# KolinGuo/MPlib

Measured on AMD Instinct MI355X. Metric: configs/sec full collide() Panda-7DoF+10 boxes, higher is better.
Workload: dtype f64; 1 GPU; cfg3 panda_10boxes: 1048576 configs/GPU/step, 129 pairs, full self+world collide() with ACM filter; configs_per_gpu=1048576, pairs=129, mask_words=5, parallelism=dp1 (config shards, no data-path collective)

## Files before the change

### mplib_amd/csrc/mpg_kernels.hip

```cpp

#include <hip/hip_runtime.h>

#include <algorithm>
#include <atomic>
#include <chrono>
#include <cfloat>
#include <cstdio>
#include <cstdlib>
#include <cstring>
#include <limits>
#include <map>
#include <memory>
#include <mutex>
#include <string>
#include <thread>
#include <vector>

#include "../../include/mpgpu.h"
#include "mpg_math.h"
#include "mpg_fk.h"
#include "mpg_hostpipe.h"

using namespace mpg;

namespace {


thread_local std::string g_last_error;

int set_error(int code, const std::string& msg) {
  g_last_error = msg;
  return code;
}

#define HIP_TRY(expr)                                                                 \
  do {                                                                                \
    hipError_t _e = (expr);                                                           \
    if (_e != hipSuccess)                                                             \
      return set_error(MPG_E_HIP, std::string(#expr " failed: ") + hipGetErrorString(_e)); \
  } while (0)




struct GObj {
  CQ4 rot, rot_inv;
  CV3 pos;
  int geom;
  int type;
};

__device__ __forceinline__ V3 hull_vertex(const DevWorld& w, cptr<double> HV, int geom, int i) {
  const cptr<double> G = HV + 12 * (size_t)(w.geom_gstart[geom] + (i >> 2)) + (i & 3);
  return v3(G[0], G[4], G[8]);
}

__device__ __forceinline__ double edot(const V3& d, const V3& p) { return (d.x * p.x + d.y * p.y) + d.z * p.z; }

__device__ __forceinline__ V3 convex_full_scan(const DevWorld& w, cptr<double> HV, int geom, const V3& dir) {
  const int g0 = w.geom_gstart[geom], ng = w.geom_ng[geom];
  const cptr<double> P = HV + 12 * (size_t)g0;
  double best = -DBL_MAX;
  int bi = 0;
  for (int g = 0; g < ng; ++g) {
    const cptr<double> G = P + 12 * g;
    double dd[4];
#pragma unroll
    for (int k = 0; k < 4; ++k) dd[k] = (dir.x * G[k] + dir.y * G[4 + k]) + dir.z * G[8 + k];
#pragma unroll
    for (int k = 0; k < 4; ++k)
      if (dd[k] > best) {
        best = dd[k];
        bi = 4 * g + k;
      }
  }
  const cptr<double> B = P + 12 * (bi >> 2) + (bi & 3);
  return v3(B[0], B[4], B[8]);
}

constexpr int kWalkWords = kMaxWalkVerts / 64;
struct WalkScratch {
  uint64_t vis[kWalkWords];
  double dd[64];
  int vi[64];
};

__device__ __forceinline__ WalkScratch& walk_scratch() {
  __shared__ WalkScratch s_walk[8];
  return s_walk[(threadIdx.x >> 6) & 7];
}

__device__ __forceinline__ void wave_lds_sync() {
  __builtin_amdgcn_fence(__ATOMIC_SEQ_CST, "wavefront");
  __builtin_amdgcn_wave_barrier();
}

__device__ __forceinline__ double lane_bcast(double v, int L) {
  const unsigned long long u = (unsigned long long)__double_as_longlong(v);
  const unsigned lo = (unsigned)__builtin_amdgcn_readlane((int)(unsigned)u, L);
  const unsigned hi = (unsigned)__builtin_amdgcn_readlane((int)(unsigned)(u >> 32), L);
  return __longlong_as_double((long long)(((unsigned long long)hi << 32) | lo));
}

__device__ __forceinline__ int big_vis_acquire(const DevWorld& w, int rank) {
  int slot = 0;
  if (rank == 0) {
    const int n = w.big_slots;
    int k = (int)((blockIdx.x * 8u + (threadIdx.x >> 6)) % (unsigned)n);
    while (atomicCAS(&w.big_busy[k], 0, 1) != 0) k = k + 1 == n ? 0 : k + 1;
    slot = k;
  }
  return __builtin_amdgcn_readfirstlane(slot);
}

__device__ __forceinline__ int wave_walk(const DevWorld& w, cptr<double> HV, int geom, const V3& d, int rank,
                                         int nact, cptr<int> pre) {
  WalkScratch& S = walk_scratch();
  const cptr<int> hd = w.hull_nbr + 2 * w.geom_nbr[geom];
  const int nwords = (w.geom_nvert[geom] + 63) >> 6;
  const bool big = nwords > kWalkWords;
  const int slot = big ? big_vis_acquire(w, rank) : -1;
  unsigned long long* vis = big ? w.big_vis + (size_t)slot * w.big_words : (unsigned long long*)S.vis;
  if (big) {
    if (rank == 0) atomicOr(&vis[0], 1ull);
    __threadfence();
  } else {
    for (int j = rank; j < nwords; j += nact)
      S.vis[j] = pre ? (uint64_t)(uint32_t)pre[4 + 2 * j] | ((uint64_t)(uint32_t)pre[5 + 2 * j] << 32) : (j == 0 ? 1ull : 0ull);
  }
  wave_lds_sync();
  int bi = pre ? pre[0] : 0, pv = pre ? pre[1] : 0, k0 = pre ? pre[2] : 0;
  bool keep = pre ? pre[3] != 0 : false, first = true;
  double best = edot(d, hull_vertex(w, HV, geom, bi));
  do {
    const int v = first ? pv : bi;
    const int skip = first ? k0 : 0;
    bool moved = first && keep;
    first = false;
    const int start = hd[2 * v] + skip, cnt = hd[2 * v + 1] - skip;
    for (int c0 = 0; c0 < cnt; c0 += nact) {
      const int m = min(cnt - c0, nact);
      if (rank < m) {
        const cptr<double> e = w.nbr_ent + 4 * (size_t)(start + c0 + rank);
        const int vi = (int)e[3];
        const uint64_t bit = 1ull << (vi & 63);
        const bool seen = (atomicOr(&vis[vi >> 6], (unsigned long long)bit) & bit) != 0ull;
        S.vi[rank] = seen ? -1 : vi;
        S.dd[rank] = seen ? 0.0 : (d.x * e[0] + d.y * e[1]) + d.z * e[2];
      }
      wave_lds_sync();
      for (int k = 0; k < m; ++k) {
        const int vi = S.vi[k];
        const double dd = S.dd[k];
        if (vi >= 0 && dd >= best) {
          moved = true;
          bi = vi;
          best = dd;
        }
      }
      wave_lds_sync();
    }
    bi = __builtin_amdgcn_readfirstlane(bi);
    keep = moved;
  } while (keep);
  if (big) {
    for (int j = rank; j < nwords; j += nact) atomicExch(&vis[j], 0ull);
    __threadfence();
    wave_lds_sync();
    if (rank == 0) atomicExch(&w.big_busy[slot], 0);
  }
  return bi;
}

// ... 799 lines not shown
    const int nk = w.n_links - w.n_free;
    for (int l = 0; l < nk; ++l) {
      const double* pl = in + (c * w.n_links + l) * 7;
      forced |= !(std::fabs(pl[0]) <= w.pose_bound && std::fabs(pl[1]) <= w.pose_bound && std::fabs(pl[2]) <= w.pose_bound);
    }
    for (int k = 0; k < w.n_free; ++k) {
      const double* pl = in + (c * w.n_links + nk + k) * 7;
      const int m = w.free_obj[k];
      const cptr<double> gr = w.geom_rec + G_STRIDE * w.moving_geom[m];
      double R[9];
      quat_to_mat(pl[3], pl[4], pl[5], pl[6], R);
      double d2 = 0.0;
#pragma unroll
      for (int i = 0; i < 3; ++i) {
        const double ci = R[3 * i] * gr[G_OBB_C] + R[3 * i + 1] * gr[G_OBB_C + 1] + R[3 * i + 2] * gr[G_OBB_C + 2] + pl[i];
        d2 += ci * ci;
      }
      if (std::sqrt(d2) - gr[G_RADIUS] > w.far_r) {
        float* r = cen + (size_t)m * 3 * BLOCK + tid;
        r[0] = kFarPark;
        r[BLOCK] = 0.f;
        r[2 * BLOCK] = 0.f;
      }
    }
  } else {
    bp_fk(w.bp, in + c * w.dof, save + tid, BLOCK, put_j);
    if (w.n_prism)
      for (int j = 0; j < w.nj; ++j)
        if (w.prism_bound[j] >= 0.0) forced |= !(std::fabs(in[c * w.dof + w.joint_q_source[j]]) <= w.prism_bound[j]);
  }
  if (w.dbg(1) || w.dbg(13)) {
    if (live && cen[tid] == 12345.f) flags[cfg] = 2;
    return;
  }

  uint32_t head = 0, tail = 0;
  uint32_t dbg_keep = 0u;
  auto push = [&](int eb, uint32_t kb) {
    if (!live) kb = 0u;
    if (w.dbg(11)) {
      dbg_keep += kb;
      return;
    }
    if (w.dbg(2)) {
      for (int i = 0; i < 32; ++i) {
        if (!((kb >> i) & 1u)) continue;
        const int p = w.sched_pair[eb + i];
        survw[(p >> 5) * BLOCK + tid] |= 1u << (p & 31);
      }
      return;
    }
    {
    const uint32_t c = (uint32_t)__popc(kb);
    uint32_t ex = 0u, total = 0u;
#pragma unroll
    for (int bit = 0; bit < 6; ++bit) {
      const unsigned long long m = __ballot((c >> bit) & 1u);
      ex += __builtin_amdgcn_mbcnt_hi((uint32_t)(m >> 32), __builtin_amdgcn_mbcnt_lo((uint32_t)m, 0u)) << bit;
      total += (uint32_t)__popcll(m) << bit;
    }
    const uint32_t incl = ex + c;
    if (total == 0u) return;
    if (tail - head + total <= (uint32_t)kQueue) {
      uint32_t pos = tail + incl - c;
      while (kb) {
        const int i = __builtin_ctz(kb);
        kb &= kb - 1u;
        queue[pos++ & (kQueue - 1)] = ((uint32_t)(eb + i) << 6) | lane;
      }
      tail += total;
      while (tail - head >= 64) {
        sat_drain<BLOCK>(w, cen, rq, cap, cfg0, survw, queue, head, 64, wbase, lane);
        head += 64;
      }
      return;
    }
    }
    uint32_t any_kb = kb;
#pragma unroll
    for (int sh = 1; sh < 64; sh <<= 1) any_kb |= (uint32_t)__shfl_xor((int)any_kb, sh);
    any_kb = __builtin_amdgcn_readfirstlane(any_kb);
    while (any_kb) {
      const int i = __builtin_ctz(any_kb);
      any_kb &= any_kb - 1u;
      const bool keep = (kb >> i) & 1u;
      const unsigned long long bal = __ballot(keep);
      if (keep) {
        const uint32_t rank =
            __builtin_amdgcn_mbcnt_hi((uint32_t)(bal >> 32), __builtin_amdgcn_mbcnt_lo((uint32_t)bal, 0u));
        queue[(tail + rank) & (kQueue - 1)] = ((uint32_t)(eb + i) << 6) | lane;
      }
      tail += (uint32_t)__popcll(bal);
      if (tail - head >= 64) {
        sat_drain<BLOCK>(w, cen, rq, cap, cfg0, survw, queue, head, 64, wbase, lane);
        head += 64;
      }
    }
  };
  const int ns = w.n_static;
  for (int g = 0; g < (FROM_POSES ? 2 : 1) && !w.dbg(12); ++g) {
    const int E0 = w.st_start[g * (ns + 1)], E1 = w.st_start[g * (ns + 1) + ns];
    if (E0 == E1) continue;
    int eb = E0;
    uint32_t kb = 0u;
    for (int sid = 0; sid < ns; ++sid) {
      const int e0 = w.st_start[g * (ns + 1) + sid], e1 = w.st_start[g * (ns + 1) + sid + 1];
      if (e0 == e1) continue;
      const cptr<float> rec = w.bp.sobj + BS_STRIDE * sid;
      float sr[BS_STRIDE];
#pragma unroll
      for (int k = 0; k < BS_STRIDE; ++k) sr[k] = rec[k];
#pragma unroll 2
      for (int e = e0; e < e1; ++e) {
        if (e - eb == 32) {
          push(eb, kb);
          eb = e;
          kb = 0u;
        }
        const float* rm = cen + (size_t)w.st_m[e] * 3 * BLOCK + tid;
        const float cm[3] = {rm[0], rm[BLOCK], rm[2 * BLOCK]};
        kb |= (uint32_t)!fsphere_obb_separated(cm, w.st_r[e], sr, w.bp_margin) << (e - eb);
      }
    }
    push(eb, kb);
  }
  for (int m = 0; m < w.n_moving; ++m) {
    const int e0 = w.sched_start[m], e1 = w.sched_start[m + 1];
    if (e0 == e1) continue;
    const float* rm = cen + (size_t)m * 3 * BLOCK + tid;
    const float cm[3] = {rm[0], rm[BLOCK], rm[2 * BLOCK]};
    const float r_m = w.bp.mobj[BM_STRIDE * m + BM_R];
    for (int eb = e0; eb < e1; eb += 32) {
      const int ee = min(e1, eb + 32);
      uint32_t kb = 0u;
#pragma unroll 4
      for (int e = eb; e < ee; ++e) {
        const int o = w.sched_other[e];
        const float* ro = cen + (size_t)o * 3 * BLOCK + tid;
        const float dx = ro[0] - cm[0], dy = ro[BLOCK] - cm[1], dz = ro[2 * BLOCK] - cm[2];
        const float rr = r_m + w.bp.mobj[BM_STRIDE * o + BM_R] + w.bp_margin;
        kb |= (uint32_t)(dx * dx + dy * dy + dz * dz <= rr * rr) << (e - eb);
      }
      push(eb, kb);
    }
  }
  if (tail != head) sat_drain<BLOCK>(w, cen, rq, cap, cfg0, survw, queue, head, tail - head, wbase, lane);
  if (forced)
    for (int k = 0; k < w.W; ++k) survw[k * BLOCK + tid] = (uint32_t)w.all_mask[k];
  if (w.dbg(8) || w.dbg(11)) {
    if (live && (survw[tid] == 12345u || dbg_keep == 12345u)) flags[cfg] = 2;
    return;
  }
  bool any = false;
  const long long tile = (cfg0 >> 6) + (tid >> 6);
  if (w.W * 8 <= kQueue) {
    uint32_t* hist = queue;
    for (int i = (int)lane; i < w.W * 8; i += 64) hist[i] = 0u;
    wave_lds_sync();
    for (int k = 0; k < w.W; ++k) {
      uint32_t x = live ? survw[k * BLOCK + tid] : 0u;
      if (live) surv[(long long)k * cap + cfg] = x;
      any |= x != 0u;
      while (x) {
        const int p = k * 32 + __builtin_ctz(x);
        x &= x - 1u;
        atomicAdd(&hist[p >> 2], 1u << (8 * (p & 3)));
      }
    }
    wave_lds_sync();
    for (int p = (int)lane; p < w.W * 32; p += 64) {
      const uint32_t c = (hist[p >> 2] >> (8 * (p & 3))) & 0xffu;
      if (c) cnt[(long long)p * n_tiles + tile] = c;
    }
  } else {
    for (int k = 0; k < w.W; ++k) {
      uint32_t x = live ? survw[k * BLOCK + tid] : 0u;
      if (live) surv[(long long)k * cap + cfg] = x;
      any |= x != 0u;
      for (;;) {
        const unsigned long long m = __ballot(x != 0u);
        if (m == 0) break;
        const uint32_t xl = __builtin_amdgcn_readlane(x, __builtin_ctzll(m));
        const int b = __builtin_ctz(xl);
        const unsigned long long bb = __ballot((x >> b) & 1u);
        x &= ~(1u << b);
        if (lane == 0) cnt[(long long)(k * 32 + b) * n_tiles + tile] = (uint32_t)__popcll(bb);
      }
    }
  }
  if (FROM_POSES || w.dbg(9)) return;
  uint32_t* list = survw + (size_t)w.W * BLOCK;
  uint32_t* wcnt = list + BLOCK;
  __syncthreads();
  const unsigned long long bal = __ballot(any);
  if (lane == 0) wcnt[tid >> 6] = (uint32_t)__popcll(bal);
  __syncthreads();
  uint32_t off = 0, total = 0;
  for (int k = 0; k < BLOCK / 64; ++k) {
    off += k < (tid >> 6) ? wcnt[k] : 0u;
    total += wcnt[k];
  }
  if (any)
    list[off + __builtin_amdgcn_mbcnt_hi((uint32_t)(bal >> 32), __builtin_amdgcn_mbcnt_lo((uint32_t)bal, 0u))] = tid;
  __syncthreads();
  if ((uint32_t)tid < total) {
    const long long r = cfg0 + list[tid];
    for (int j = 0; j < w.nj; ++j) {
      const int src = w.joint_q_source[j];
      if (src < 0 || !joint_is_revolute(w.joint_type[j])) continue;
      double sv, cv;
      mpg_sincos(in[r * w.dof + src], &sv, &cv);
      sc[(r * w.dof + src) * 2] = sv;
      sc[(r * w.dof + src) * 2 + 1] = cv;
    }
  }
}

__global__ __launch_bounds__(1024) void pair_scan_kernel(uint32_t* __restrict__ cnt, int n_tiles,
                                                        uint32_t* __restrict__ seg_len) {
  __shared__ uint32_t part[16];
  uint32_t* c = cnt + (long long)blockIdx.x * n_tiles;
  const int per = (n_tiles + 1023) / 1024;
  const int lo = threadIdx.x * per, hi = min(n_tiles, lo + per);
  const uint32_t lane = threadIdx.x & 63u, wv = threadIdx.x >> 6;
  uint32_t v[16];
  uint32_t sum = 0;
  if (per <= 16) {
#pragma unroll
    for (int k = 0; k < 16; ++k) {
      v[k] = lo + k < hi ? c[lo + k] : 0u;
      sum += v[k];
    }
  } else {
    for (int i = lo; i < hi; ++i) sum += c[i];
  }
  const uint32_t incl = wave_inclusive_scan(sum, lane);
  if (lane == 63u) part[wv] = incl;
  __syncthreads();
  uint32_t pre = 0, tot = 0;
#pragma unroll
  for (uint32_t k = 0; k < 16; ++k) {
    const uint32_t x = part[k];
    pre += k < wv ? x : 0u;
    tot += x;
  }
  uint32_t run = pre + incl - sum;
  if (per <= 16) {
#pragma unroll
    for (int k = 0; k < 16; ++k) {
      if (lo + k < hi) c[lo + k] = run;
      run += v[k];
    }
  } else {
    for (int i = lo; i < hi; ++i) {
      const uint32_t x = c[i];
      c[i] = run;
      run += x;
    }
  }
  if (threadIdx.x == 0) seg_len[blockIdx.x] = tot;
}

#ifndef MPG_TASK_MIN
#define MPG_TASK_MIN 8
#endif
constexpr uint32_t kTaskMin = MPG_TASK_MIN;

__device__ __forceinline__ uint32_t block_sum256(uint32_t v, uint32_t* red) {
#pragma unroll
  for (int off = 32; off > 0; off >>= 1) v += __shfl_xor(v, off);
  __syncthreads();
  if ((threadIdx.x & 63u) == 0) red[threadIdx.x >> 6] = v;
  __syncthreads();
  return red[0] + red[1] + red[2] + red[3];
}

__global__ __launch_bounds__(256) void chunk_scan_kernel(const uint32_t* __restrict__ seg_len, int n_pairs,
                                                        uint32_t* __restrict__ seg_start,
                                                        uint32_t* __restrict__ prefix, unsigned long long* units,
                                                        uint32_t target_tasks) {
  __shared__ uint32_t wl[4], wt[4], red[4];
  const uint32_t lane = threadIdx.x & 63u, wv = threadIdx.x >> 6;
  uint32_t part = 0;
  for (int p = (int)threadIdx.x; p < n_pairs; p += 256) part += seg_len[p];
  const uint32_t all = block_sum256(part, red);
  uint32_t ts = target_tasks ? (all + target_tasks - 1) / target_tasks : kTask;
  ts = ts < kTaskMin ? kTaskMin : (ts > kTask ? kTask : ts);
  ts = (ts + 7u) & ~7u;
  uint32_t cl = 0, ct = 0;
  for (int p0 = 0; p0 < n_pairs; p0 += 256) {
    const int p = p0 + (int)threadIdx.x;
    const uint32_t len = p < n_pairs ? seg_len[p] : 0u;
    const uint32_t tasks = (len + ts - 1) / ts;
    const uint32_t il = wave_inclusive_scan(len, lane), it = wave_inclusive_scan(tasks, lane);
    if (lane == 63) {
      wl[wv] = il;
      wt[wv] = it;
    }
    __syncthreads();
    uint32_t bl = cl, bt = ct;
    for (uint32_t k = 0; k < wv; ++k) {
      bl += wl[k];
      bt += wt[k];
    }
    if (p < n_pairs) {
      seg_start[p] = bl + il - len;
      prefix[p] = bt + it - tasks;
    }
    for (uint32_t k = 0; k < 4; ++k) {
      cl += wl[k];
      ct += wt[k];
    }
    __syncthreads();
  }
  if (threadIdx.x == 0) {
    prefix[n_pairs] = ct;
    prefix[n_pairs + 1] = 0;
    prefix[n_pairs + 2] = ts;
    prefix[n_pairs + 3] = cl;
    if (units) atomicAdd(units, (unsigned long long)cl);
  }
}

__global__ __launch_bounds__(256) void scatter_kernel(const uint32_t* __restrict__ surv, long long n, long long cap,
                                                     int n_pairs, int W, int n_tiles,
                                                     const uint32_t* __restrict__ off,
                                                     const uint32_t* __restrict__ seg_start,
                                                     uint32_t* __restrict__ cand) {
  const uint32_t lane = lane_id();
  const long long wid = __builtin_amdgcn_readfirstlane((blockIdx.x * blockDim.x + threadIdx.x) >> 6);
  if (wid >= (long long)n_tiles * W) return;
  const int wd = (int)(wid / n_tiles), t = (int)(wid % n_tiles);
  const long long cfg = (long long)t * 64 + lane;
  const uint32_t x = cfg < n ? surv[(long long)wd * cap + cfg] : 0u;
  uint32_t o = x;
#pragma unroll
  for (int sh = 1; sh < 64; sh <<= 1) o |= (uint32_t)__shfl_xor((int)o, sh);
  o = __builtin_amdgcn_readfirstlane(o);
  if (o == 0u) return;
  uint32_t base = 0u;
  if (lane < 32u && ((o >> lane) & 1u)) {
    const int p = wd * 32 + (int)lane;
    base = seg_start[p] + off[(long long)p * n_tiles + t];
  }
  for (uint32_t m = o; m; m &= m - 1u) {
    const int b = __builtin_ctz(m);
    const uint32_t bit = (x >> b) & 1u;
    const unsigned long long bal = __ballot(bit);
    const uint32_t bs = __builtin_amdgcn_readlane(base, b);
    if (bit)
      cand[bs + __builtin_amdgcn_mbcnt_hi((uint32_t)(bal >> 32), __builtin_amdgcn_mbcnt_lo((uint32_t)bal, 0u))] =
          (uint32_t)cfg;
  }
}

__device__ __forceinline__ int task_pair(const uint32_t* __restrict__ prefix, int n_pairs, uint32_t tk) {
  int lo = 0, hi = n_pairs;
  while (hi - lo > 1) {
    const int mid = (lo + hi) >> 1;
    if (prefix[mid] <= tk) lo = mid;
    else hi = mid;
  }
  return lo;
}

enum : int { MPR_DONE = 0, MPR_V1 = 1, MPR_V2 = 2, MPR_V3 = 3, MPR_V4 = 4 };

__device__ __forceinline__ bool octree_wave(const DevWorld& w, cptr<double> HV, int go, const SE3& TO, int gs,
                                           const SE3& TS);

template <int CLS>
__device__ __forceinline__ unsigned long long walk_wave_eval(const DevWorld& w, cptr<double> HV, int ga, const SE3& TA,
                                                            int gb, const SE3& TB, bool active);

template <int CLS>
__device__ __forceinline__ bool pair_closed_form(int cf, const DevWorld& w, int ga, const SE3& TA, int gb,
                                                 const SE3& TB) {
  if constexpr (CLS == CLS_CLOSED) return closed_form(cf, w, ga, TA, gb, TB);
  if constexpr (CLS == CLS_GJK) return gjk_indep_intersect(w, ga, TA, gb, TB);
  return false;
}

template <bool FROM_POSES, int CLS>
__global__ __launch_bounds__(256, CLS == CLS_OCTREE ? 2 : 1) void closed_form_kernel(DevWorld w, const double* __restrict__ in,
                                                         const uint32_t* __restrict__ seg_len,
                                                         const uint32_t* __restrict__ seg_start,
                                                         const uint32_t* __restrict__ prefix,
                                                         const uint32_t* __restrict__ cand,
                                                         uint8_t* __restrict__ flags, uint32_t* __restrict__ masks,
                                                         const double* __restrict__ sc) {
  const uint32_t lane = lane_id();
  const uint32_t wave = __builtin_amdgcn_readfirstlane((blockIdx.x * blockDim.x + threadIdx.x) >> 6);
  const uint32_t n_waves = (gridDim.x * blockDim.x) >> 6;
  const uint32_t total = prefix[w.n_pairs];
  for (uint32_t tk = wave; tk < total; tk += n_waves) {
    int lo = 0, hi = w.n_pairs;
    while (hi - lo > 1) {
      const int mid = (lo + hi) >> 1;
      if (prefix[mid] <= tk) lo = mid;
      else hi = mid;
    }
    const int p = lo;
    const int cf = w.pair_cf[p];
    if (cf == CF_NONE || cf_class(cf) != CLS) continue;
    const uint32_t ts = prefix[w.n_pairs + 2];
    const uint32_t t0 = (tk - prefix[p]) * ts, t1 = min(seg_len[p], t0 + ts);
    const int a = w.pair_a[p], b = w.pair_b[p];
    const bool am = a < w.n_moving, bm = b < w.n_moving;
    const int ga = am ? w.moving_geom[a] : w.static_geom[a - w.n_moving];
    const int gb = bm ? w.moving_geom[b] : w.static_geom[b - w.n_moving];
    const uint32_t* __restrict__ cl = cand + seg_start[p];
    for (uint32_t base = t0; base < t1; base += 64) {
      const uint32_t idx = base + lane;
      if constexpr (CLS == CLS_OCTREE || CLS == CLS_MESH) {
        const bool active = idx < t1;
        const long long c = active ? cl[idx] : 0;
        SE3 TA = {}, TB = {};
        if (active) {
          TA = am ? moving_tf<FROM_POSES>(w, in, sc, c, a) : load_se3(w.static_T + 12 * (a - w.n_moving));
          TB = bm ? moving_tf<FROM_POSES>(w, in, sc, c, b) : load_se3(w.static_T + 12 * (b - w.n_moving));
        }
        const unsigned long long hits = walk_wave_eval<CLS>(w, w.hull, ga, TA, gb, TB, active);
        if ((hits >> lane) & 1ull) {
          if (masks) atomicOr(&masks[c * w.W + (p >> 5)], 1u << (p & 31));
          flags[c] = 1;
        }
        continue;
      }
      if (idx >= t1) continue;
      const long long c = cl[idx];
      const SE3 TA = am ? moving_tf<FROM_POSES>(w, in, sc, c, a) : load_se3(w.static_T + 12 * (a - w.n_moving));
      const SE3 TB = bm ? moving_tf<FROM_POSES>(w, in, sc, c, b) : load_se3(w.static_T + 12 * (b - w.n_moving));
      if (pair_closed_form<CLS>(cf, w, ga, TA, gb, TB)) {
        if (masks) atomicOr(&masks[c * w.W + (p >> 5)], 1u << (p & 31));
        flags[c] = 1;
      }
    }
  }
}

__device__ __forceinline__ int mpr_advance(ccd_real mpr_tol, const CV3& s, int& st_io, CV3& v0_io, CV3& v1_io, CV3& v2_io,
                                           CV3& v3_io, CV3& dir_io) {
  int st = st_io;
  CV3 v0 = v0_io, v1 = v1_io, v2 = v2_io, v3 = v3_io, dir = dir_io;
  int res = 0;
  const ccd_real dsd = vdot(s, dir);
  CV3 ca, cb;
  bool post_swap = false, post_encl = false;
  if (st == MPR_V4) {
    if (!(is_zero(dsd) || dsd > 0)) {
      res = -1;
    } else {
      const ccd_real dv1 = vdot(v1, dir), dv2 = vdot(v2, dir), dv3 = vdot(v3, dir);
      ccd_real d1 = dsd - dv1;
      const ccd_real dd2 = dsd - dv2, dd3 = dsd - dv3;
      d1 = (d1 < dd2) ? d1 : dd2;
      d1 = (d1 < dd3) ? d1 : dd3;
      if (ccd_eq(d1, mpr_tol) || d1 < mpr_tol) {
        res = -1;
      } else {
        const CV3 v4v0 = vcross(s, v0);
        if (vdot(v1, v4v0) > 0) {
          if (vdot(v2, v4v0) > 0) v1 = s;
          else v3 = s;
        } else {
          if (vdot(v3, v4v0) > 0) v2 = s;
          else v1 = s;
        }
        ca = vsub(v2, v1);
        cb = vsub(v3, v1);
        post_encl = true;
      }
    }
  } else if (is_zero(dsd) || dsd < 0) {
    res = -1;
  } else if (st == MPR_V1) {
    v1 = s;
    ca = v0;
    cb = v1;
  } else if (st == MPR_V2) {
    v2 = s;
    ca = vsub(v1, v0);
    cb = vsub(v2, v0);
    post_swap = true;
  } else {
    v3 = s;
    bool cont = false;
    ccd_real d2 = vdot(vcross(v1, v3), v0);
    if (d2 < 0 && !is_zero(d2)) {
      v2 = v3;
      cont = true;
    }
    if (!cont) {
      d2 = vdot(vcross(v3, v2), v0);
      if (d2 < 0 && !is_zero(d2)) {
        v1 = v3;
        cont = true;
      }
// ... 4562 lines not shown
```

### mplib_amd/csrc/mpg_streams_host.h

```cpp
#pragma once

void release_stream_locked(mpg_world* w, hipStream_t s) {
  const auto wi = w->ws.find(s);
  const auto si = w->sides.find(s);
  if (wi == w->ws.end() && si == w->sides.end()) return;
  hipDeviceSynchronize();
  if (wi != w->ws.end()) w->ws.erase(wi);
  if (si != w->sides.end()) {
    w->ws.erase(si->second.side.get());
    w->sides.erase(si);
  }
}

void evict_streams_locked(mpg_world* w) {
  std::map<hipStream_t, uint64_t> callers;
  for (auto& kv : w->ws) callers[kv.first] = kv.second.last;
  for (auto& kv : w->sides) {
    callers.erase(kv.second.side.get());
    uint64_t& t = callers[kv.first];
    t = std::max(t, kv.second.last);
  }
  for (auto& kv : w->busy)
    if (kv.second > 0) callers.erase(kv.first);
  size_t pinned = 0;
  for (auto& kv : w->busy) pinned += kv.second > 0;
  while (!callers.empty() && callers.size() + pinned >= mpg_world::kMaxStreamState) {
    auto lru = callers.begin();
    for (auto it = callers.begin(); it != callers.end(); ++it)
      if (it->second < lru->second) lru = it;
    release_stream_locked(w, lru->first);
    callers.erase(lru);
  }
}

struct StreamPin {
  mpg_world* w;
  hipStream_t s;
  StreamPin(mpg_world* w_, hipStream_t s_) : w(w_), s(s_) {
    std::lock_guard<std::mutex> lk(w->ws_mu);
    ++w->busy[s];
  }
  ~StreamPin() {
    std::lock_guard<std::mutex> lk(w->ws_mu);
    if (--w->busy[s] <= 0) w->busy.erase(s);
  }
};

bool is_side_stream_locked(const mpg_world* w, hipStream_t s) {
  for (auto& kv : w->sides)
    if (kv.second.side.get() == s) return true;
  return false;
}

int get_workspace(mpg_world* w, hipStream_t s, long long want, mpg_world::Workspace** out) {
  std::lock_guard<std::mutex> lk(w->ws_mu);
  if (w->ws.find(s) == w->ws.end() && !is_side_stream_locked(w, s) && w->sides.find(s) == w->sides.end())
    evict_streams_locked(w);
  auto& ws = w->ws[s];
  ws.last = ++w->ws_tick;
  const long long np = std::max(w->dw.n_pairs, 1);
  if (ws.cap < want) {
    ws = mpg_world::Workspace{};
    ws.last = w->ws_tick;
    const long long tiles = (want + 63) / 64;
    HIP_TRY(ws.surv.reserve((size_t)w->dw.W * want));
    HIP_TRY(ws.cnt.reserve((size_t)np * tiles));
    HIP_TRY(ws.seg_len.reserve(np));
    HIP_TRY(ws.seg_start.reserve(np));
    HIP_TRY(ws.prefix.reserve(np + 4));
    HIP_TRY(ws.cand.reserve((size_t)np * want));
    HIP_TRY(ws.rq.reserve((size_t)4 * std::max(w->dw.n_moving, 1) * want));
    HIP_TRY(ws.sc.reserve((size_t)2 * std::max(w->dw.dof, 1) * want));
    ws.cap = want;
  }
  *out = &ws;
  return MPG_OK;
}

Event prof_event(mpg_world* w) {
  Event e;
  if (!w->ev_pool.empty()) {
    e = std::move(w->ev_pool.back());
    w->ev_pool.pop_back();
  } else {
    e.create(hipEventDefault);
  }
  return e;
}

struct StageTimer {
  mpg_world* w;
  hipStream_t s;
  int stage;
  Event a;
  StageTimer(mpg_world* w_, hipStream_t s_, int st) : w(w_), s(s_), stage(st) {
    if (!w->prof) return;
    std::lock_guard<std::mutex> lk(w->prof_mu);
    a = prof_event(w);
    if (a) hipEventRecord(a.get(), s);
  }
  void stop() {
    if (!a) return;
    std::lock_guard<std::mutex> lk(w->prof_mu);
    Event b = prof_event(w);
    if (!b) return;
    hipEventRecord(b.get(), s);
    w->marks.push_back({stage, std::move(a), std::move(b)});
  }
  ~StageTimer() { stop(); }
};

struct ContactOut {
  double *depth, *normal, *pos;
};

template <bool FROM_POSES>
int launch_collide(mpg_world* w, const double* in, long long n, uint8_t* flags, uint32_t* masks, hipStream_t stream,
                   const ContactOut* co = nullptr) {
  if (n == 0) return MPG_OK;
  StreamPin pin(w, stream);
  const long long chunk = std::min<long long>(n, w->max_chunk);
  mpg_world::Workspace* owner = nullptr;
  int rc = get_workspace(w, stream, chunk, &owner);
  if (rc) return rc;
  uint32_t *const surv = owner->surv.get(), *const cnt = owner->cnt.get(), *const seg_len = owner->seg_len.get(),
                  *const seg_start = owner->seg_start.get(), *const prefix = owner->prefix.get(),
                  *const cand = owner->cand.get();
  float* const rq = owner->rq.get();
  double* const sc = owner->sc.get();
  const long long cap = owner->cap;
  const size_t row = FROM_POSES ? (size_t)w->dw.n_links * 7 : (size_t)w->dw.dof;
  for (long long off = 0; off < n; off += chunk) {
    const long long m = std::min(chunk, n - off);
    const double* qin = in + off * row;
    uint8_t* fl = flags + off;
    uint32_t* mk = masks ? masks + off * w->dw.W : nullptr;
    const unsigned grid = (unsigned)((m + w->block - 1) / w->block);
    const int n_tiles = (int)((m + 63) / 64);
    StageTimer t_cull(w, stream, MPG_STAGE_CULL);
    if (w->prof) w->prof_cfg += m;
    HIP_TRY(hipMemsetAsync(cnt, 0, sizeof(uint32_t) * std::max(w->dw.n_pairs, 1) * (size_t)n_tiles, stream));
    switch (w->block) {
      case 256:
        hipLaunchKernelGGL((cull_kernel<256, FROM_POSES>), dim3(grid), dim3(256), w->lds_bytes, stream, w->dw, qin,
                           m, fl, mk, surv, rq, sc, cap, cnt, n_tiles);
        break;
      case 128:
        hipLaunchKernelGGL((cull_kernel<128, FROM_POSES>), dim3(grid), dim3(128), w->lds_bytes, stream, w->dw, qin,
                           m, fl, mk, surv, rq, sc, cap, cnt, n_tiles);
        break;
      default:
        hipLaunchKernelGGL((cull_kernel<64, FROM_POSES>), dim3(grid), dim3(64), w->lds_bytes, stream, w->dw, qin, m,
                           fl, mk, surv, rq, sc, cap, cnt, n_tiles);
        break;
    }
    HIP_TRY(hipGetLastError());
    t_cull.stop();
    StageTimer t_bucket(w, stream, MPG_STAGE_BUCKET);
    const long long tw = (long long)n_tiles * w->dw.W;
    const unsigned gb = (unsigned)((tw + 3) / 4);
    if (w->dw.n_pairs > 0) {
      hipLaunchKernelGGL(pair_scan_kernel, dim3(w->dw.n_pairs), dim3(1024), 0, stream, cnt, n_tiles, seg_len);
      HIP_TRY(hipGetLastError());
    }
    hipLaunchKernelGGL(chunk_scan_kernel, dim3(1), dim3(256), 0, stream, seg_len, w->dw.n_pairs, seg_start,
                       prefix, w->prof ? w->prof_units.get() : nullptr, (uint32_t)(4 * w->narrow_blocks));
    HIP_TRY(hipGetLastError());
    hipLaunchKernelGGL(scatter_kernel, dim3(gb), dim3(256), 0, stream, surv, m, cap, w->dw.n_pairs, w->dw.W,
                       n_tiles, cnt, seg_start, cand);
    HIP_TRY(hipGetLastError());
    t_bucket.stop();
    StageTimer t_narrow(w, stream, MPG_STAGE_NARROW);
    const long long want_waves = (m * std::max(w->dw.n_pairs, 1) + kTaskMin - 1) / kTaskMin;
    const unsigned nb = (unsigned)std::max<long long>(1, std::min<long long>(w->narrow_blocks, (want_waves + 3) / 4));
    hipLaunchKernelGGL((narrow_kernel<FROM_POSES>), dim3(nb), dim3(256), 0, stream, w->dw, qin, seg_len,
                       seg_start, prefix, cand, fl, mk, prefix + w->dw.n_pairs + 1, sc);
    HIP_TRY(hipGetLastError());
    if (w->any_closed_form) {
      hipLaunchKernelGGL((closed_form_kernel<FROM_POSES, CLS_CLOSED>), dim3(w->narrow_blocks), dim3(256), 0, stream,
                         w->dw, qin, seg_len, seg_start, prefix, cand, fl, mk, sc);
      HIP_TRY(hipGetLastError());
    }
    if (w->any_octree) {
      hipLaunchKernelGGL((closed_form_kernel<FROM_POSES, CLS_OCTREE>), dim3(w->narrow_blocks), dim3(256), 0, stream,
                         w->dw, qin, seg_len, seg_start, prefix, cand, fl, mk, sc);
      HIP_TRY(hipGetLastError());
    }
    if (w->any_mesh) {
      hipLaunchKernelGGL((closed_form_kernel<FROM_POSES, CLS_MESH>), dim3(w->narrow_blocks), dim3(256), 0, stream,
                         w->dw, qin, seg_len, seg_start, prefix, cand, fl, mk, sc);
      HIP_TRY(hipGetLastError());
    }
    if (w->any_gjk) {
      hipLaunchKernelGGL((closed_form_kernel<FROM_POSES, CLS_GJK>), dim3(w->narrow_blocks), dim3(256), 0, stream,
                         w->dw, qin, seg_len, seg_start, prefix, cand, fl, mk, sc);
      HIP_TRY(hipGetLastError());
    }
    if (co) {
      const size_t P = (size_t)w->dw.n_pairs;
      HIP_TRY(hipMemsetAsync(co->depth + off * P, 0, sizeof(double) * m * P, stream));
      HIP_TRY(hipMemsetAsync(co->normal + off * P * 3, 0, sizeof(double) * m * P * 3, stream));
      HIP_TRY(hipMemsetAsync(co->pos + off * P * 3, 0, sizeof(double) * m * P * 3, stream));
      hipLaunchKernelGGL((contact_kernel<FROM_POSES>), dim3(nb), dim3(256), 0, stream, w->dw, qin, seg_len,
                         seg_start, prefix, cand, mk, sc, co->depth + off * P, co->normal + off * P * 3,
                         co->pos + off * P * 3);
      HIP_TRY(hipGetLastError());
    }
  }
  return MPG_OK;
}

int ensure_staging(mpg_world* w, size_t ncfg, size_t nout) {
  if (ncfg > w->cap_cfg) {
    w->d_q.reset();
    w->d_flags.reset();
    w->d_masks.reset();
    w->cap_cfg = 0;
    HIP_TRY(w->d_q.reserve(std::max<size_t>(1, ncfg * std::max(w->dw.dof, 1))));
    HIP_TRY(w->d_flags.reserve(std::max<size_t>(1, ncfg)));
    HIP_TRY(w->d_masks.reserve(std::max<size_t>(1, ncfg * w->dw.W)));
    w->cap_cfg = ncfg;
  }
  if (nout > w->cap_out) {
    w->cap_out = 0;
    HIP_TRY(w->d_out.reserve(nout));
    w->cap_out = nout;
  }
  return MPG_OK;
}

int scratch_begin(Event& last, hipStream_t s) {
  if (!last) HIP_TRY(last.create(hipEventDisableTiming));
  else HIP_TRY(hipStreamWaitEvent(s, last.get(), 0));
  return MPG_OK;
}
template <class T>
int scratch_grow(const Event& last, DevBuf<T>& buf, size_t n) {
  if (buf.get() && buf.cap() < n && last) HIP_TRY(hipEventSynchronize(last.get()));
  HIP_TRY(buf.reserve(n));
  return MPG_OK;
}

int ensure_ring(mpg_world* w, size_t cap, size_t row) {
  auto& R = w->ring;
  if (!R.h2d) {
    HIP_TRY(R.h2d.create(hipStreamNonBlocking));
    HIP_TRY(R.side.create(hipStreamNonBlocking));
    for (int j = 0; j < mpg_world::kRing; ++j) {
      HIP_TRY(R.e_in[j].create(hipEventDisableTiming));
      HIP_TRY(R.e_done[j].create(hipEventDisableTiming));
    }
  }
  const size_t in = cap * std::max<size_t>(row, 1);
  if (cap <= R.cap && in <= R.in_cap) return MPG_OK;
  cap = std::max(cap, R.cap);
  const size_t in_cap = std::max(in, R.in_cap);
  for (auto& S : R.slot) S = mpg_world::Ring::Slot{};
  R.cap = R.in_cap = 0;
  const size_t W = (size_t)std::max(w->dw.W, 1);
  const size_t blocks = (cap + kPackCfg - 1) / kPackCfg;
  for (auto& S : R.slot) {
    HIP_TRY(S.d_in.reserve(in_cap));
    HIP_TRY(S.d_fl.reserve(cap));
    HIP_TRY(S.d_mk.reserve(W * cap));
    HIP_TRY(S.d_bcnt.reserve(blocks));
    HIP_TRY(S.h_fl.reserve(cap, kPinMapped));
    HIP_TRY(S.h_mk.reserve(W * cap, kPinMapped));
    HIP_TRY(S.h_bcnt.reserve(blocks, kPinMapped));
  }
  R.cap = cap;
  R.in_cap = in_cap;
  return MPG_OK;
}
```

### mplib_amd/csrc/mpg_world.h

```cpp
#pragma once

struct mpg_world {
  ~mpg_world();
  int device = 0;
  DevWorld dw{};
  int n_geoms = 0;
  std::vector<int> geom_type_h;
  DevBuf<char> blob;
  size_t blob_bytes = 0;
  uint64_t snapshot_hash = 0;
  Stream own_stream;
  Event gather_ev;
  DevBuf<unsigned long long> big_vis;
  DevBuf<int> big_busy;
  DevBuf<unsigned long long> stats;
  DevBuf<double> free_dev;
  int block = 128;
  size_t lds_bytes = 0;
  std::mutex host_mu;
  DevBuf<double> d_q, d_out;
  DevBuf<uint8_t> d_flags;
  DevBuf<uint32_t> d_masks;
  size_t cap_cfg = 0;
  size_t cap_out = 0;
  struct Workspace {
    DevBuf<uint32_t> surv;
    DevBuf<uint32_t> cnt;
    DevBuf<uint32_t> seg_len;
    DevBuf<uint32_t> seg_start;
    DevBuf<uint32_t> prefix;
    DevBuf<uint32_t> cand;
    DevBuf<float> rq;
    DevBuf<double> sc;
    DevBuf<double> links;
    long long links_cap = 0;
    long long cap = 0;
    uint64_t last = 0;
  };
  struct Side {
    Stream side;
    Event fork, join;
    uint64_t last = 0;
  };
  std::mutex ws_mu;
  std::map<hipStream_t, Side> sides;
  std::map<hipStream_t, Workspace> ws;
  std::vector<double> free_host;
  struct FreeStage {
    DevBuf<double> q, fp, links;
    DevBuf<uint8_t> fl;
    DevBuf<uint32_t> mk;
  } free_stage;
  struct Mark {
    int stage;
    Event a, b;
  };
  struct Motion {
    Event last;
    DevBuf<double> edges;
    DevBuf<int32_t> segs;
    DevBuf<long long> offs;
    DevBuf<char> out;
    DevBuf<double> states;
    DevBuf<uint8_t> flags;
    DevBuf<double> fp;
    DevBuf<int32_t> row_of;
  } motion;
  std::mutex motion_mu;
  bool has_closed_form = false;
  bool has_octree = false;
  bool octree_first = false;
  bool any_closed_form = false;
  bool any_octree = false;
  bool has_mesh = false;
  bool any_mesh = false;
  bool any_gjk = false;
  bool has_octree2 = false;
  struct Dist {
    Event last;
    DevBuf<double> poses, save64, q;
    DevBuf<char> out;
    DevBuf<double> pts;
    DevBuf<double> links;
    DevBuf<double> fp;
    DevBuf<ccdx::BigPolytope> big;
    DevBuf<unsigned> list;
  } dist;
  struct ContactStage {
    DevBuf<double> in, out;
    DevBuf<uint8_t> fl;
    DevBuf<uint32_t> mk;
    DevBuf<double> fp;
  } contact;
  std::mutex dist_mu;
  std::mutex prof_mu;
  bool prof = false;
  std::vector<Mark> marks;
  std::vector<Event> ev_pool;
  double prof_ms[MPG_NUM_STAGES] = {0, 0, 0};
  int64_t prof_n[MPG_NUM_STAGES] = {0, 0, 0};
  int64_t prof_cfg = 0;
  DevBuf<unsigned long long> prof_units;
  long long max_chunk = 1 << 20;
  int narrow_blocks = 1024;
  long long overlap_min = 1 << 18;
  int overlap_parts = 2;
  static constexpr size_t kMaxStreamState = 32;
  uint64_t ws_tick = 0;
  std::map<hipStream_t, int> busy;
  long long small_max = 1024;
  struct Small {
    PinnedBuf<double> h_q;
    PinnedBuf<uint8_t> h_hits;
    DevBuf<double> d_qs;
    DevBuf<double> d_ssc;
    PinnedBuf<double> h_ssc;
  } small;
  int64_t small_host_sc = 64;
  bool small_args = true;
  std::vector<int> h_rev_src;
  bool small_zero_copy = true;
  int64_t small_inline_sc = 256;
  Stream srv_stream;
  PinnedBuf<SrvCtl> srv;
  unsigned long long srv_seq = 0;
  bool srv_running = false;
  bool srv_ok = false;
  bool srv_broken = false;
  std::chrono::steady_clock::time_point srv_retry_at{};
  bool srv_quitting = false;
  int64_t srv_served = 0, srv_starts = 0, srv_fallbacks = 0;
  int srv_mode = 1;
  long long srv_idle_us = 1000;
  int srv_g = 8;
  int srv_max_n = kSrvN;
  size_t srv_lds = 0;
  bool srv_stats = false;
  double srv_stat[8] = {0, 0, 0, 0, 0, 0, 0, 0};
  size_t small_cap = 0;
  size_t small_qcap = 0;
  static constexpr int kRing = 3;
  struct Ring {
    Stream h2d;
    Stream side;
    Event e_in[kRing], e_done[kRing];
    struct Slot {
      DevBuf<double> d_in;
      DevBuf<uint8_t> d_fl;
      DevBuf<uint32_t> d_mk;
      DevBuf<uint32_t> d_bcnt;
      PinnedBuf<uint8_t> h_fl;
      PinnedBuf<uint32_t> h_mk;
      PinnedBuf<uint32_t> h_bcnt;
    } slot[kRing];
    size_t cap = 0;
    size_t in_cap = 0;
  } ring;
  long long ring_chunk = 1 << 19;
  int ring_streams = 2;
  int host_threads = 8;
  long long ring_head = 1 << 17, ring_tail = 1 << 16;
  std::unique_ptr<mpg_hostpipe::Pool> pool;
  double hp_stat[6] = {0, 0, 0, 0, 0, 0};
};
```

Measured before the change: 1.551 billion configs/s.

## Store per-tile pair counts as byte rows and scan them hierarchically

```diff
diff --git a/mplib_amd/csrc/mpg_bucket.h b/mplib_amd/csrc/mpg_bucket.h
--- /dev/null
+++ b/mplib_amd/csrc/mpg_bucket.h
@@ -0,0 +1,45 @@
+#pragma once
+
+#include "mpg_math.h"
+
+#ifndef MPG_RANGE_TILES
+#define MPG_RANGE_TILES 8
+#endif
+
+namespace mpg {
+
+constexpr int kRangeTiles = MPG_RANGE_TILES;
+constexpr int kGroupRanges = 16;
+static_assert(64 * kRangeTiles * kGroupRanges < 65536, "a group's count of one pair must fit 16 bits");
+
+MPG_INLINE int bk_row_words(int W) { return W * 8; }
+MPG_INLINE int bk_cols(int W) { return W * 32; }
+MPG_INLINE long long bk_tiles(long long n) { return (n + 63) / 64; }
+MPG_INLINE int bk_ranges(int n_tiles) { return (n_tiles + kRangeTiles - 1) / kRangeTiles; }
+MPG_INLINE int bk_groups(int n_ranges) { return (n_ranges + kGroupRanges - 1) / kGroupRanges; }
+MPG_INLINE int bk_range_first(int r) { return r * kRangeTiles; }
+MPG_INLINE int bk_range_end(int r, int n_tiles) {
+  const int e = (r + 1) * kRangeTiles;
+  return e < n_tiles ? e : n_tiles;
+}
+MPG_INLINE int bk_group_first(int g) { return g * kGroupRanges; }
+MPG_INLINE int bk_group_end(int g, int n_ranges) {
+  const int e = (g + 1) * kGroupRanges;
+  return e < n_ranges ? e : n_ranges;
+}
+MPG_INLINE int bk_group_of(int r) { return r / kGroupRanges; }
+constexpr int kSumSlots = 4096;
+MPG_INLINE bool bk_fold_sum(int n_ranges, int W) { return (long long)n_ranges * bk_row_words(W) <= kSumSlots; }
+MPG_INLINE long long bk_wave_tile(long long block_idx, int block, int tid) {
+  return ((block_idx * block) >> 6) + (tid >> 6);
+}
+MPG_INLINE bool bk_tile_has_row(long long tile, int n_tiles) { return tile < (long long)n_tiles; }
+MPG_INLINE size_t bk_cnt_words(int W, long long cap) { return (size_t)bk_tiles(cap) * (size_t)bk_row_words(W); }
+MPG_INLINE size_t bk_part_words(int W, long long cap) {
+  return (size_t)bk_ranges((int)bk_tiles(cap)) * (size_t)bk_cols(W);
+}
+MPG_INLINE size_t bk_grp_words(int W, long long cap) {
+  return (size_t)bk_groups(bk_ranges((int)bk_tiles(cap))) * (size_t)bk_cols(W);
+}
+
+}
diff --git a/mplib_amd/csrc/mpg_kernels.hip b/mplib_amd/csrc/mpg_kernels.hip
--- a/mplib_amd/csrc/mpg_kernels.hip
+++ b/mplib_amd/csrc/mpg_kernels.hip
@@ -19,6 +19,7 @@
 #include "../../include/mpgpu.h"
 #include "mpg_math.h"
 #include "mpg_fk.h"
+#include "mpg_bucket.h"
 #include "mpg_hostpipe.h"
 
 using namespace mpg;
@@ -1124,7 +1125,8 @@
     return;
   }
   bool any = false;
-  const long long tile = (cfg0 >> 6) + (tid >> 6);
+  const long long tile = bk_wave_tile(blockIdx.x, BLOCK, tid);
+  const bool has_row = bk_tile_has_row(tile, n_tiles);
   if (w.W * 8 <= kQueue) {
     uint32_t* hist = queue;
     for (int i = (int)lane; i < w.W * 8; i += 64) hist[i] = 0u;
@@ -1140,9 +1142,9 @@
       }
     }
     wave_lds_sync();
-    for (int p = (int)lane; p < w.W * 32; p += 64) {
-      const uint32_t c = (hist[p >> 2] >> (8 * (p & 3))) & 0xffu;
-      if (c) cnt[(long long)p * n_tiles + tile] = c;
+    if (has_row) {
+      uint32_t* row = cnt + tile * bk_row_words(w.W);
+      for (int i = (int)lane; i < bk_row_words(w.W); i += 64) row[i] = hist[i];
     }
   } else {
     for (int k = 0; k < w.W; ++k) {
@@ -1156,7 +1158,8 @@
         const int b = __builtin_ctz(xl);
         const unsigned long long bb = __ballot((x >> b) & 1u);
         x &= ~(1u << b);
-        if (lane == 0) cnt[(long long)(k * 32 + b) * n_tiles + tile] = (uint32_t)__popcll(bb);
+        if (lane == 0 && has_row)
+          reinterpret_cast<uint8_t*>(cnt)[tile * bk_cols(w.W) + k * 32 + b] = (uint8_t)__popcll(bb);
       }
     }
   }
@@ -1188,49 +1191,54 @@
   }
 }
 
-__global__ __launch_bounds__(1024) void pair_scan_kernel(uint32_t* __restrict__ cnt, int n_tiles,
-                                                        uint32_t* __restrict__ seg_len) {
-  __shared__ uint32_t part[16];
-  uint32_t* c = cnt + (long long)blockIdx.x * n_tiles;
-  const int per = (n_tiles + 1023) / 1024;
-  const int lo = threadIdx.x * per, hi = min(n_tiles, lo + per);
-  const uint32_t lane = threadIdx.x & 63u, wv = threadIdx.x >> 6;
-  uint32_t v[16];
-  uint32_t sum = 0;
-  if (per <= 16) {
-#pragma unroll
-    for (int k = 0; k < 16; ++k) {
-      v[k] = lo + k < hi ? c[lo + k] : 0u;
-      sum += v[k];
-    }
-  } else {
-    for (int i = lo; i < hi; ++i) sum += c[i];
-  }
-  const uint32_t incl = wave_inclusive_scan(sum, lane);
-  if (lane == 63u) part[wv] = incl;
-  __syncthreads();
-  uint32_t pre = 0, tot = 0;
-#pragma unroll
-  for (uint32_t k = 0; k < 16; ++k) {
-    const uint32_t x = part[k];
-    pre += k < wv ? x : 0u;
-    tot += x;
-  }
-  uint32_t run = pre + incl - sum;
-  if (per <= 16) {
-#pragma unroll
-    for (int k = 0; k < 16; ++k) {
-      if (lo + k < hi) c[lo + k] = run;
-      run += v[k];
-    }
-  } else {
-    for (int i = lo; i < hi; ++i) {
-      const uint32_t x = c[i];
-      c[i] = run;
-      run += x;
-    }
-  }
-  if (threadIdx.x == 0) seg_len[blockIdx.x] = tot;
+constexpr int kSumCols = 256;
+static_assert(kGroupRanges * kSumCols <= kSumSlots, "a group's sums must fit the block's LDS");
+
+template <int NT>
+__device__ __forceinline__ void range_sum_groups(const uint32_t* __restrict__ cnt, int n_tiles, int W,
+                                                 uint32_t* __restrict__ part, uint32_t* __restrict__ grp, int g0,
+                                                 int ng, uint2* sums) {
+  const int rw = bk_row_words(W), C = bk_cols(W);
+  const int n_ranges = bk_ranges(n_tiles);
+  const int r0 = bk_group_first(g0), nr = bk_group_end(g0 + ng - 1, n_ranges) - r0;
+  for (int j0 = 0; j0 < rw; j0 += kSumCols) {
+    const int jc = min(kSumCols, rw - j0);
+    for (int i = threadIdx.x; i < nr * jc; i += NT) {
+      const int rl = i / jc, jl = i % jc;
+      const int t0 = bk_range_first(r0 + rl), t1 = bk_range_end(r0 + rl, n_tiles);
+      const uint32_t* col = cnt + j0 + jl;
+      uint32_t lo = 0, hi = 0;
+#pragma unroll
+      for (int k = 0; k < kRangeTiles; ++k) {
+        const uint32_t x = t0 + k < t1 ? col[(long long)(t0 + k) * rw] : 0u;
+        lo += x & 0x00ff00ffu;
+        hi += (x >> 8) & 0x00ff00ffu;
+      }
+      sums[i] = make_uint2(lo, hi);
+    }
+    __syncthreads();
+    for (int i = threadIdx.x; i < ng * jc; i += NT) {
+      const int gl = i / jc, jl = i % jc;
+      const int rl1 = bk_group_end(g0 + gl, n_ranges) - r0;
+      uint32_t lo = 0, hi = 0;
+      for (int rl = bk_group_first(gl); rl < rl1; ++rl) {
+        *reinterpret_cast<uint4*>(part + (long long)(r0 + rl) * C + 4 * (j0 + jl)) =
+            make_uint4(lo & 0xffffu, hi & 0xffffu, lo >> 16, hi >> 16);
+        const uint2 s = sums[rl * jc + jl];
+        lo += s.x;
+        hi += s.y;
+      }
+      *reinterpret_cast<uint4*>(grp + (long long)(g0 + gl) * C + 4 * (j0 + jl)) =
+          make_uint4(lo & 0xffffu, hi & 0xffffu, lo >> 16, hi >> 16);
+    }
+    __syncthreads();
+  }
+}
+
+__global__ __launch_bounds__(256) void range_sum_kernel(const uint32_t* __restrict__ cnt, int n_tiles, int W,
+                                                       uint32_t* __restrict__ part, uint32_t* __restrict__ grp) {
+  __shared__ uint2 sums[kSumSlots];
+  range_sum_groups<256>(cnt, n_tiles, W, part, grp, blockIdx.x, 1, sums);
 }
 
 #ifndef MPG_TASK_MIN
@@ -1238,31 +1246,94 @@
 #endif
 constexpr uint32_t kTaskMin = MPG_TASK_MIN;
 
-__device__ __forceinline__ uint32_t block_sum256(uint32_t v, uint32_t* red) {
+constexpr int kScanRegs = 24;
+
+__device__ __forceinline__ uint32_t block_sum1024(uint32_t v, uint32_t* red) {
 #pragma unroll
   for (int off = 32; off > 0; off >>= 1) v += __shfl_xor(v, off);
   __syncthreads();
   if ((threadIdx.x & 63u) == 0) red[threadIdx.x >> 6] = v;
   __syncthreads();
-  return red[0] + red[1] + red[2] + red[3];
-}
-
-__global__ __launch_bounds__(256) void chunk_scan_kernel(const uint32_t* __restrict__ seg_len, int n_pairs,
-                                                        uint32_t* __restrict__ seg_start,
-                                                        uint32_t* __restrict__ prefix, unsigned long long* units,
-                                                        uint32_t target_tasks) {
-  __shared__ uint32_t wl[4], wt[4], red[4];
+  uint32_t s = 0;
+#pragma unroll
+  for (int k = 0; k < 16; ++k) s += red[k];
+  return s;
+}
+
+__global__ __launch_bounds__(1024) void range_scan_kernel(const uint32_t* __restrict__ cnt, int n_tiles, int W,
+                                                         uint32_t* __restrict__ part, uint32_t* __restrict__ grp,
+                                                         int n_groups, int n_pairs, uint32_t* seg_len,
+                                                         uint32_t* __restrict__ seg_start,
+                                                         uint32_t* __restrict__ prefix, unsigned long long* units,
+                                                         uint32_t target_tasks) {
+  __shared__ uint2 sums[kSumSlots];
+  __shared__ uint32_t wl[16], wt[16], red[16];
+  uint32_t* slab = reinterpret_cast<uint32_t*>(sums);
+  const int tid = threadIdx.x;
   const uint32_t lane = threadIdx.x & 63u, wv = threadIdx.x >> 6;
-  uint32_t part = 0;
-  for (int p = (int)threadIdx.x; p < n_pairs; p += 256) part += seg_len[p];
-  const uint32_t all = block_sum256(part, red);
+  const int C = bk_cols(W);
+  if (cnt) range_sum_groups<1024>(cnt, n_tiles, W, part, grp, 0, n_groups, sums);
+  const bool one = C <= 1024;
+  uint32_t my_len = 0;
+  {
+    const int CP = min(C, 1024), S = 1024 / CP, per = (n_groups + S - 1) / S;
+    const int s = tid / CP, cl = tid % CP;
+    for (int c0 = 0; c0 < C; c0 += CP) {
+      const int col = c0 + cl;
+      const bool act = s < S && col < C;
+      const int lo = s * per, hi = act ? min(n_groups, lo + per) : lo;
+      const uint32_t i0 = (uint32_t)lo * C + col;
+      uint32_t v[kScanRegs];
+      uint32_t sum = 0;
+      if (per <= kScanRegs) {
+#pragma unroll
+        for (int k = 0; k < kScanRegs; ++k) {
+          v[k] = lo + k < hi ? grp[i0 + (uint32_t)k * C] : 0u;
+          sum += v[k];
+        }
+      } else {
+        for (int i = lo; i < hi; ++i) sum += grp[i0 + (uint32_t)(i - lo) * C];
+      }
+      slab[tid] = sum;
+      __syncthreads();
+      uint32_t run = 0, tot = 0;
+      for (int k = 0; k < S; ++k) {
+        const uint32_t x = slab[k * CP + cl];
+        run += k < s ? x : 0u;
+        tot += x;
+      }
+      if (per <= kScanRegs) {
+#pragma unroll
+        for (int k = 0; k < kScanRegs; ++k) {
+          if (lo + k < hi) grp[i0 + (uint32_t)k * C] = run;
+          run += v[k];
+        }
+      } else {
+        for (int i = lo; i < hi; ++i) {
+          const uint32_t x = grp[i0 + (uint32_t)(i - lo) * C];
+          grp[i0 + (uint32_t)(i - lo) * C] = run;
+          run += x;
+        }
+      }
+      if (act && s == 0 && col < n_pairs) {
+        seg_len[col] = tot;
+        my_len = tot;
+      }
+      __syncthreads();
+    }
+  }
+  uint32_t psum = 0;
+  if (one) psum = my_len;
+  else
+    for (int p = tid; p < n_pairs; p += 1024) psum += seg_len[p];
+  const uint32_t all = block_sum1024(psum, red);
   uint32_t ts = target_tasks ? (all + target_tasks - 1) / target_tasks : kTask;
   ts = ts < kTaskMin ? kTaskMin : (ts > kTask ? kTask : ts);
   ts = (ts + 7u) & ~7u;
   uint32_t cl = 0, ct = 0;
-  for (int p0 = 0; p0 < n_pairs; p0 += 256) {
-    const int p = p0 + (int)threadIdx.x;
-    const uint32_t len = p < n_pairs ? seg_len[p] : 0u;
+  for (int p0 = 0; p0 < n_pairs; p0 += 1024) {
+    const int p = p0 + tid;
+    const uint32_t len = one ? my_len : (p < n_pairs ? seg_len[p] : 0u);
     const uint32_t tasks = (len + ts - 1) / ts;
     const uint32_t il = wave_inclusive_scan(len, lane), it = wave_inclusive_scan(tasks, lane);
     if (lane == 63) {
@@ -1279,7 +1350,7 @@
       seg_start[p] = bl + il - len;
       prefix[p] = bt + it - tasks;
     }
-    for (uint32_t k = 0; k < 4; ++k) {
+    for (uint32_t k = 0; k < 16; ++k) {
       cl += wl[k];
       ct += wt[k];
     }
@@ -1296,26 +1367,30 @@
 
 __global__ __launch_bounds__(256) void scatter_kernel(const uint32_t* __restrict__ surv, long long n, long long cap,
                                                      int n_pairs, int W, int n_tiles,
-                                                     const uint32_t* __restrict__ off,
+                                                     const uint32_t* __restrict__ cnt,
+                                                     const uint32_t* __restrict__ part,
+                                                     const uint32_t* __restrict__ grp,
                                                      const uint32_t* __restrict__ seg_start,
                                                      uint32_t* __restrict__ cand) {
   const uint32_t lane = lane_id();
   const long long wid = __builtin_amdgcn_readfirstlane((blockIdx.x * blockDim.x + threadIdx.x) >> 6);
   if (wid >= (long long)n_tiles * W) return;
-  const int wd = (int)(wid / n_tiles), t = (int)(wid % n_tiles);
+  const int wd = (int)(wid % W), t = (int)(wid / W);
+  const int r = t / kRangeTiles, t0 = bk_range_first(r);
+  const int C = bk_cols(W);
   const long long cfg = (long long)t * 64 + lane;
   const uint32_t x = cfg < n ? surv[(long long)wd * cap + cfg] : 0u;
-  uint32_t o = x;
-#pragma unroll
-  for (int sh = 1; sh < 64; sh <<= 1) o |= (uint32_t)__shfl_xor((int)o, sh);
-  o = __builtin_amdgcn_readfirstlane(o);
-  if (o == 0u) return;
-  uint32_t base = 0u;
-  if (lane < 32u && ((o >> lane) & 1u)) {
+  uint32_t c = 0u, base = 0u;
+  if (lane < 32u) {
     const int p = wd * 32 + (int)lane;
-    base = seg_start[p] + off[(long long)p * n_tiles + t];
-  }
-  for (uint32_t m = o; m; m &= m - 1u) {
+    const uint8_t* c8 = reinterpret_cast<const uint8_t*>(cnt) + p;
+    c = c8[(long long)t * C];
+    uint32_t pre = 0u;
+#pragma unroll
+    for (int k = 0; k < kRangeTiles - 1; ++k) pre += t0 + k < t ? c8[(long long)(t0 + k) * C] : 0u;
+    if (p < n_pairs) base = seg_start[p] + grp[(long long)bk_group_of(r) * C + p] + part[(long long)r * C + p] + pre;
+  }
+  for (uint32_t m = (uint32_t)__ballot(c != 0u); m; m &= m - 1u) {
     const int b = __builtin_ctz(m);
     const uint32_t bit = (x >> b) & 1u;
     const unsigned long long bal = __ballot(bit);
diff --git a/mplib_amd/csrc/mpg_streams_host.h b/mplib_amd/csrc/mpg_streams_host.h
--- a/mplib_amd/csrc/mpg_streams_host.h
+++ b/mplib_amd/csrc/mpg_streams_host.h
@@ -62,9 +62,10 @@
   if (ws.cap < want) {
     ws = mpg_world::Workspace{};
     ws.last = w->ws_tick;
-    const long long tiles = (want + 63) / 64;
     HIP_TRY(ws.surv.reserve((size_t)w->dw.W * want));
-    HIP_TRY(ws.cnt.reserve((size_t)np * tiles));
+    HIP_TRY(ws.cnt.reserve(bk_cnt_words(w->dw.W, want)));
+    HIP_TRY(ws.part.reserve(bk_part_words(w->dw.W, want)));
+    HIP_TRY(ws.grp.reserve(bk_grp_words(w->dw.W, want)));
     HIP_TRY(ws.seg_len.reserve(np));
     HIP_TRY(ws.seg_start.reserve(np));
     HIP_TRY(ws.prefix.reserve(np + 4));
@@ -123,7 +124,8 @@
   mpg_world::Workspace* owner = nullptr;
   int rc = get_workspace(w, stream, chunk, &owner);
   if (rc) return rc;
-  uint32_t *const surv = owner->surv.get(), *const cnt = owner->cnt.get(), *const seg_len = owner->seg_len.get(),
+  uint32_t *const surv = owner->surv.get(), *const cnt = owner->cnt.get(), *const part = owner->part.get(),
+                  *const grp = owner->grp.get(), *const seg_len = owner->seg_len.get(),
                   *const seg_start = owner->seg_start.get(), *const prefix = owner->prefix.get(),
                   *const cand = owner->cand.get();
   float* const rq = owner->rq.get();
@@ -139,7 +141,10 @@
     const int n_tiles = (int)((m + 63) / 64);
     StageTimer t_cull(w, stream, MPG_STAGE_CULL);
     if (w->prof) w->prof_cfg += m;
-    HIP_TRY(hipMemsetAsync(cnt, 0, sizeof(uint32_t) * std::max(w->dw.n_pairs, 1) * (size_t)n_tiles, stream));
+#ifndef MPG_DIAG
+    if (w->dw.W * 8 > kQueue)
+#endif
+      HIP_TRY(hipMemsetAsync(cnt, 0, sizeof(uint32_t) * bk_cnt_words(w->dw.W, m), stream));
     switch (w->block) {
       case 256:
         hipLaunchKernelGGL((cull_kernel<256, FROM_POSES>), dim3(grid), dim3(256), w->lds_bytes, stream, w->dw, qin,
@@ -157,17 +162,20 @@
     HIP_TRY(hipGetLastError());
     t_cull.stop();
     StageTimer t_bucket(w, stream, MPG_STAGE_BUCKET);
+    const int n_ranges = bk_ranges(n_tiles), n_groups = bk_groups(n_ranges);
     const long long tw = (long long)n_tiles * w->dw.W;
     const unsigned gb = (unsigned)((tw + 3) / 4);
-    if (w->dw.n_pairs > 0) {
-      hipLaunchKernelGGL(pair_scan_kernel, dim3(w->dw.n_pairs), dim3(1024), 0, stream, cnt, n_tiles, seg_len);
-      HIP_TRY(hipGetLastError());
-    }
-    hipLaunchKernelGGL(chunk_scan_kernel, dim3(1), dim3(256), 0, stream, seg_len, w->dw.n_pairs, seg_start,
-                       prefix, w->prof ? w->prof_units.get() : nullptr, (uint32_t)(4 * w->narrow_blocks));
+    const bool fold = bk_fold_sum(n_ranges, w->dw.W);
+    if (!fold) {
+      hipLaunchKernelGGL(range_sum_kernel, dim3(n_groups), dim3(256), 0, stream, cnt, n_tiles, w->dw.W, part, grp);
+      HIP_TRY(hipGetLastError());
+    }
+    hipLaunchKernelGGL(range_scan_kernel, dim3(1), dim3(1024), 0, stream, fold ? cnt : nullptr, n_tiles, w->dw.W,
+                       part, grp, n_groups, w->dw.n_pairs, seg_len, seg_start, prefix,
+                       w->prof ? w->prof_units.get() : nullptr, (uint32_t)(4 * w->narrow_blocks));
     HIP_TRY(hipGetLastError());
     hipLaunchKernelGGL(scatter_kernel, dim3(gb), dim3(256), 0, stream, surv, m, cap, w->dw.n_pairs, w->dw.W,
-                       n_tiles, cnt, seg_start, cand);
+                       n_tiles, cnt, part, grp, seg_start, cand);
     HIP_TRY(hipGetLastError());
     t_bucket.stop();
     StageTimer t_narrow(w, stream, MPG_STAGE_NARROW);
diff --git a/mplib_amd/csrc/mpg_world.h b/mplib_amd/csrc/mpg_world.h
--- a/mplib_amd/csrc/mpg_world.h
+++ b/mplib_amd/csrc/mpg_world.h
@@ -26,6 +26,8 @@
   struct Workspace {
     DevBuf<uint32_t> surv;
     DevBuf<uint32_t> cnt;
+    DevBuf<uint32_t> part;
+    DevBuf<uint32_t> grp;
     DevBuf<uint32_t> seg_len;
     DevBuf<uint32_t> seg_start;
     DevBuf<uint32_t> prefix;
```

Result: faster. 1.588 billion configs/s, median of 6 (+2.4%).
